# allenai/embodied-clip

Measured on AMD Instinct MI355X. Metric: env-frames/sec (CLIP encode + policy fwd/bwd + PPO update), higher is better.
Workload: dtype bf16

## Files before the change

embodied_clip_amd/csrc/api.hip:

```cpp
#include <stdlib.h>

#include "common.h"

extern "C" int ec_version(void) { return 610; }

extern "C" const char* ec_strerror(int code) {
    switch (code) {
        case EC_OK: return "ok";
        case EC_ERR_ARG: return "invalid argument (null pointer or bad enum)";
        case EC_ERR_SHAPE: return "unsupported shape for this kernel";
        case EC_ERR_LAUNCH: return "HIP kernel launch failed";
        case EC_ERR_WORKSPACE: return "workspace too small";
        case EC_ERR_ALLOC: return "host allocation failed";
        case EC_ERR_UNSUPPORTED: return "unsupported configuration";
        default: return "unknown error";
    }
}

namespace {
int env_int(const char* name, int dflt) {
    const char* e = getenv(name);
    return e ? atoi(e) : dflt;
}
EcConfig read_config() {
    EcConfig c;
    c.conv_narrow = env_int("EC_CONV_NARROW", 3);
    c.conv_rowsn = env_int("EC_CONV_ROWSN", 1);
    c.conv_big = env_int("EC_CONV_BIG", 1);
    c.conv8_min_tiles = env_int("EC_CONV8_MIN_TILES", 0);
    c.conv8_bn128 = env_int("EC_CONV8_BN128", 0);
    c.conv8_longseg = env_int("EC_CONV8_LONGSEG", 1);
    c.conv_t224 = env_int("EC_CONV_T224", 2);
    c.conv_t64 = env_int("EC_CONV_T64", 150);
    c.conv_ring = env_int("EC_CONV_RING", 1);
    c.conv_regw = env_int("EC_CONV_REGW", 1);
    c.rn50_fuse = env_int("EC_RN50_FUSE", 1);
    c.rn50_bneck = env_int("EC_RN50_BNECK", 128);
    c.rn50_bneck3 = env_int("EC_RN50_BNECK3", 1);
    c.rn50_img3 = env_int("EC_RN50_IMG3", 1);
    c.rn50_dscat = env_int("EC_RN50_DSCAT", 1);
    c.rn50_poolout = env_int("EC_RN50_POOLOUT", 1);
    c.gemm_no_x3 = env_int("EC_GEMM_NO_X3", 0);
    c.gemm_bwd3 = env_int("EC_GEMM_BWD3", 0);
    c.policy_fast = env_int("EC_POLICY_FAST", 1);
    c.act_split = env_int("EC_ACT_SPLIT", 1);
    c.tail_fused = env_int("EC_TAIL_FUSED", 1);
    c.gru_fused = env_int("EC_GRU_FUSED", 2);
    c.c1_pingpong = env_int("EC_C1_PINGPONG", 1);
    c.dw1_tr = env_int("EC_DW1_TR", 1);
    c.wih_perm = env_int("EC_WIH_PERM", 1);
    c.dw_transposed = env_int("EC_DW_TRANSPOSED", 1);
    c.vit_wide = env_int("EC_VIT_WIDE", 1);
    c.vit_bm192 = env_int("EC_VIT_BM192", 1);
    return c;
}
}

const EcConfig& ec_config() {
    static const EcConfig c = read_config();
    return c;
}

uint64_t ec_config_hash() {
    const EcConfig& c = ec_config();
    uint64_t x = 1469598103934665603ull;
    auto mix = [&](long v) {
        for (int i = 0; i < 8; ++i) { x ^= (uint64_t)((v >> (8 * i)) & 0xff); x *= 1099511628211ull; }
    };
    mix(c.conv_narrow); mix(c.conv_rowsn); mix(c.conv_big); mix(c.conv8_min_tiles); mix(c.conv8_bn128); mix(c.conv8_longseg);
    mix(c.conv_t224); mix(c.conv_t64); mix(c.conv_ring); mix(c.conv_regw); mix(c.rn50_fuse); mix(c.rn50_bneck); mix(c.rn50_bneck3);
    mix(c.rn50_img3); mix(c.rn50_dscat); mix(c.rn50_poolout); mix(c.gemm_no_x3); mix(c.gemm_bwd3); mix(c.policy_fast); mix(c.act_split); mix(c.tail_fused); mix(c.gru_fused); mix(c.c1_pingpong);
    mix(c.dw1_tr); mix(c.wih_perm); mix(c.dw_transposed);
    return x;
}

namespace {
__global__ void spin_kernel(unsigned long long ticks) {
    const unsigned long long t0 = __builtin_amdgcn_s_memrealtime();
    while (__builtin_amdgcn_s_memrealtime() - t0 < ticks) __builtin_amdgcn_s_sleep(16);
}
}

extern "C" int ec_bind_streams(ec_stream_t* streams, int n, int spin_us) {
    if (!streams || n <= 0 || spin_us <= 0 || spin_us > 100000) return EC_ERR_ARG;
    if (hipDeviceSynchronize() != hipSuccess) return EC_ERR_LAUNCH;
    for (int round = 0; round < 2; ++round)
        for (int i = 0; i < n; ++i)
            hipLaunchKernelGGL(spin_kernel, dim3(1), dim3(64), 0, (hipStream_t)streams[i], (unsigned long long)spin_us * 100ull);
    EC_CHECK_LAUNCH();
    return hipDeviceSynchronize() == hipSuccess ? EC_OK : EC_ERR_LAUNCH;
}

extern "C" int ec_stream_pair_overlap(ec_stream_t a, ec_stream_t b, int spin_us, float* ratio) {
    if (!ratio || spin_us <= 0 || spin_us > 100000 || a == b) return EC_ERR_ARG;
    hipStream_t sa = (hipStream_t)a, sb = (hipStream_t)b;
    hipEvent_t e[4];
    for (auto& ev : e)
        if (hipEventCreate(&ev) != hipSuccess) return EC_ERR_LAUNCH;
    const unsigned long long ticks = (unsigned long long)spin_us * 100ull;
    float best = 1e30f;
    int rc = EC_OK;
    for (int rep = 0; rep < 3 && rc == EC_OK; ++rep) {
        float alone = 0.f, both = 0.f;
        if (hipDeviceSynchronize() != hipSuccess) { rc = EC_ERR_LAUNCH; break; }
        (void)hipEventRecord(e[0], sa);
        hipLaunchKernelGGL(spin_kernel, dim3(1), dim3(64), 0, sa, ticks);
        (void)hipEventRecord(e[1], sa);
        if (hipDeviceSynchronize() != hipSuccess) { rc = EC_ERR_LAUNCH; break; }
        (void)hipEventRecord(e[2], sa);
        (void)hipStreamWaitEvent(sb, e[2], 0);
        hipLaunchKernelGGL(spin_kernel, dim3(1), dim3(64), 0, sa, ticks);
        hipLaunchKernelGGL(spin_kernel, dim3(1), dim3(64), 0, sb, ticks);
        (void)hipEventRecord(e[3], sb);
        (void)hipStreamWaitEvent(sa, e[3], 0);
        (void)hipEventRecord(e[1], sa);
        if (hipDeviceSynchronize() != hipSuccess) { rc = EC_ERR_LAUNCH; break; }
        if (hipEventElapsedTime(&both, e[2], e[1]) != hipSuccess) { rc = EC_ERR_LAUNCH; break; }
        (void)hipEventRecord(e[0], sa);
        hipLaunchKernelGGL(spin_kernel, dim3(1), dim3(64), 0, sa, ticks);
        (void)hipEventRecord(e[3], sa);
        if (hipDeviceSynchronize() != hipSuccess) { rc = EC_ERR_LAUNCH; break; }
        if (hipEventElapsedTime(&alone, e[0], e[3]) != hipSuccess || alone <= 0.f) { rc = EC_ERR_LAUNCH; break; }
        best = both / alone < best ? both / alone : best;
    }
    for (auto& ev : e) (void)hipEventDestroy(ev);
    if (rc == EC_OK) *ratio = best;
    return rc;
}
```

embodied_clip_amd/csrc/conv3x3_narrow.hip:

```cpp
#include <stdlib.h>

#include <type_traits>
#include <utility>

#include "common.h"

namespace {

typedef unsigned int u32x4 __attribute__((ext_vector_type(4)));
constexpr int PX = 32;
__device__ u32x4 ec_zero_page3[4];

struct N3Args {
    const uint16_t *in, *w;
    const float* bias;
    uint16_t* out;
    int H, W, ntiles;
    unsigned in_bytes = 0;
    int dbg = 0;
};

__device__ __forceinline__ float dppq_xor1(float v) {
    return __builtin_bit_cast(float, __builtin_amdgcn_update_dpp(0, __builtin_bit_cast(int, v), 0xB1, 0xF, 0xF, true));
}
__device__ __forceinline__ float dppq_xor2(float v) {
    return __builtin_bit_cast(float, __builtin_amdgcn_update_dpp(0, __builtin_bit_cast(int, v), 0x4E, 0xF, 0xF, true));
}
__device__ __forceinline__ float relu1(float x) { return __builtin_amdgcn_fmed3f(x, 0.f, __builtin_inff()); }
__device__ __forceinline__ int wunit(int n, int hh) { return ((2 * n + hh) ^ ((n >> 3) & 1)) << 4; }

template <int CIN, int COUT, bool POOL, int NW>
__global__ __launch_bounds__(NW * 64, 1) void conv3x3_narrow_kernel(N3Args p) {
    constexpr int KSTEPS = 9 * CIN / 16;
    constexpr int CB = CIN / 16;
    constexpr int FN = COUT / 32;
    constexpr int K = 9 * CIN;
    constexpr int W_BYTES = KSTEPS * COUT * 32;
    constexpr int OP = COUT * 2 + 16;
    constexpr int STG = (POOL ? PX / 4 : PX) * OP;
    extern __shared__ __attribute__((aligned(16))) unsigned char sm[];
    float* sB = reinterpret_cast<float*>(sm + W_BYTES);
    const int tid = threadIdx.x, lane = tid & 63, wave = tid >> 6;
    unsigned char* stg = sm + W_BYTES + COUT * 4 + wave * STG;
    const int px = lane & 31, h = lane >> 5;

    ec_stage_all<COUT * (K / 8), NW * 64, u32x4>(
        tid,
        [&](int idx) { return *reinterpret_cast<const u32x4*>(p.w + (long)(idx / (K / 8)) * K + (idx % (K / 8)) * 8); },
        [&](int idx, const u32x4& v) {
            const int n = idx / (K / 8), c = idx % (K / 8);
            *reinterpret_cast<u32x4*>(sm + (c >> 1) * (COUT * 32) + wunit(n, c & 1)) = v;
        });
    for (int i = tid; i < COUT; i += NW * 64) sB[i] = p.bias[i];
    __syncthreads();

    const int GW = gridDim.x * NW;
    const unsigned char* in_b = reinterpret_cast<const unsigned char*>(p.in);
    const unsigned char* zp = reinterpret_cast<const unsigned char*>(ec_zero_page3);
    const int HW = p.H * p.W;

    const int lb = (int)ec_xcd_remap(blockIdx.x, gridDim.x);
    for (int t = lb * NW + wave; t < p.ntiles; t += GW) {
        const int m = t * PX + px;
        int y, x, pix;
        if (POOL) {
            const int q = m >> 2, s2 = m & 3;
            const int Hp = p.H >> 1, Wp = p.W >> 1;
            const int b = q / (Hp * Wp);
            const int r2 = q - b * (Hp * Wp);
            const int yp = r2 / Wp;
            y = 2 * yp + (s2 >> 1);
            x = 2 * (r2 - yp * Wp) + (s2 & 1);
            pix = (b * p.H + y) * p.W + x;
        } else {
            const int b = m / HW;
            const int r2 = m - b * HW;
            y = r2 / p.W;
            x = r2 - y * p.W;
            pix = m;
        }
        const unsigned xm = (x > 0 ? 1u : 0u) | 2u | (x < p.W - 1 ? 4u : 0u);
        const unsigned msk = (y > 0 ? xm : 0u) | (xm << 3) | (y < p.H - 1 ? (xm << 6) : 0u);
        const unsigned char* base = in_b + ((long)pix * CIN + h * 8) * 2;

        f32x16_t acc[FN];
#pragma unroll
        for (int n = 0; n < FN; ++n)
#pragma unroll
            for (int r = 0; r < 16; ++r) acc[n][r] = 0.f;
        constexpr int PH = (KSTEPS + 17) / 18, PS = KSTEPS / PH;
        static_assert(PS * PH == KSTEPS, "phase split");
        auto phase = [&](auto phc) {
            constexpr int S0 = decltype(phc)::value * PS;
            u32x4 a[PS];
            [&]<int... I>(std::integer_sequence<int, I...>) {
                ((a[I] = *reinterpret_cast<const u32x4*>(
                      ((msk >> ((S0 + I) / CB)) & 1u)
                          ? base + (((((S0 + I) / CB) / 3 - 1) * p.W + (((S0 + I) / CB) % 3 - 1)) * CIN + ((S0 + I) % CB) * 16) * 2
                          : zp + h * 16)),
                 ...);
            }(std::make_integer_sequence<int, PS>{});
            __builtin_amdgcn_sched_barrier(0);
            [&]<int... I>(std::integer_sequence<int, I...>) {
                (([&] {
                     const bf16x8_t aop = __builtin_bit_cast(bf16x8_t, a[I]);
#pragma unroll
                     for (int n = 0; n < FN; ++n) {
                         const s16x8_t wf = *reinterpret_cast<const s16x8_t*>(sm + (S0 + I) * (COUT * 32) + wunit(32 * n + px, h));
                         acc[n] = __builtin_amdgcn_mfma_f32_32x32x16_bf16(__builtin_bit_cast(bf16x8_t, wf), aop, acc[n], 0, 0, 0);
                     }
                 }()),
                 ...);
            }(std::make_integer_sequence<int, PS>{});
            __builtin_amdgcn_sched_barrier(0);
        };
        [&]<int... P>(std::integer_sequence<int, P...>) { (phase(std::integral_constant<int, P>{}), ...); }
        (std::make_integer_sequence<int, PH>{});

#pragma unroll
        for (int n = 0; n < FN; ++n)
#pragma unroll
            for (int g = 0; g < 4; ++g) {
                const int lc = 32 * n + 8 * g + 4 * h;
                const float4 bv = *reinterpret_cast<const float4*>(sB + lc);
                float v0 = fmaxf(acc[n][4 * g + 0] + bv.x, 0.f), v1 = fmaxf(acc[n][4 * g + 1] + bv.y, 0.f);
                float v2 = fmaxf(acc[n][4 * g + 2] + bv.z, 0.f), v3 = fmaxf(acc[n][4 * g + 3] + bv.w, 0.f);
                if (POOL) {
                    v0 += dppq_xor1(v0); v1 += dppq_xor1(v1); v2 += dppq_xor1(v2); v3 += dppq_xor1(v3);
                    v0 += dppq_xor2(v0); v1 += dppq_xor2(v1); v2 += dppq_xor2(v2); v3 += dppq_xor2(v3);
                    if ((lane & 3) == 0) {
                        uint2 o;
                        o.x = ec_pack2(0.25f * v0, 0.25f * v1);
                        o.y = ec_pack2(0.25f * v2, 0.25f * v3);
                        *reinterpret_cast<uint2*>(stg + (px >> 2) * OP + lc * 2) = o;
                    }
                } else {
                    uint2 o;
                    o.x = ec_pack2(v0, v1);
                    o.y = ec_pack2(v2, v3);
                    *reinterpret_cast<uint2*>(stg + px * OP + lc * 2) = o;
                }
            }
        constexpr int ORows = POOL ? PX / 4 : PX;
        constexpr int ZC = COUT / 8;
        const long orow0 = (long)t * ORows;
#pragma unroll
        for (int i = 0; i < (ORows * ZC + 63) / 64; ++i) {
            const int idx = i * 64 + lane;
            if (ORows * ZC >= 64 || idx < ORows * ZC) {
                const u32x4 v = *reinterpret_cast<const u32x4*>(stg + (idx / ZC) * OP + (idx % ZC) * 16);
                *reinterpret_cast<u32x4*>(p.out + (orow0 + idx / ZC) * COUT + (idx % ZC) * 8) = v;
            }
        }
    }
}


template <int CIN, int COUT, bool POOL, int NW>
__global__ __launch_bounds__(NW * 64, 1) void conv3x3_rows_kernel(N3Args p) {
    constexpr int KSTEPS = 9 * CIN / 16, CB = CIN / 16, FN = COUT / 32, K = 9 * CIN;
    constexpr int CPP = CIN / 8;
    constexpr int PITCH = CIN * 2 + 16;
    constexpr int RW = POOL ? 16 : 30;
    constexpr int RPB = POOL ? RW * PITCH + 128 : RW * PITCH;
    constexpr int NR = POOL ? 4 : 3;
    constexpr int REGION = NR * RPB + 4 * PITCH;
    constexpr int NCH = NR * RW * CPP;
    constexpr int IT = (NCH + 63) / 64;
    constexpr int W_BYTES = KSTEPS * COUT * 32;
    constexpr int OP = COUT * 2 + 16;
    extern __shared__ __attribute__((aligned(16))) unsigned char sm[];
    float* sB = reinterpret_cast<float*>(sm + W_BYTES);
    const int tid = threadIdx.x, lane = tid & 63, wave = tid >> 6;
    unsigned char* img = sm + W_BYTES + COUT * 4 + wave * REGION;
    const int px = lane & 31, h = lane >> 5;

    ec_stage_all<COUT * (K / 8), NW * 64, u32x4>(
        tid,
        [&](int idx) { return *reinterpret_cast<const u32x4*>(p.w + (long)(idx / (K / 8)) * K + (idx % (K / 8)) * 8); },
        [&](int idx, const u32x4& v) {
            const int n = idx / (K / 8), c = idx % (K / 8);
            *reinterpret_cast<u32x4*>(sm + (c >> 1) * (COUT * 32) + wunit(n, c & 1)) = v;
        });
    for (int i = tid; i < COUT; i += NW * 64) sB[i] = p.bias[i];
    __syncthreads();

    const int GW = gridDim.x * NW;
    const int lb = (int)ec_xcd_remap(blockIdx.x, gridDim.x);
    const int nseg = POOL ? p.W / 14 : p.W / 28;
    const int nrow = POOL ? p.H / 2 : p.H;

    int f_r[IT], f_px[IT], f_lds[IT], f_goff[IT];
#pragma unroll
    for (int i = 0; i < IT; ++i) {
        const int g = i * 64 + lane;
        const int r = g / (RW * CPP), rem = g - r * (RW * CPP);
        f_r[i] = (g < NCH) ? r : -100000;
        f_px[i] = rem / CPP;
        f_lds[i] = r * RPB + (rem / CPP) * PITCH + (rem % CPP) * 16;
        f_goff[i] = ((r * p.W + rem / CPP) * CIN + (rem % CPP) * 8) * 2;
    }
    int obase;
    if (POOL) obase = ((px >> 1) & 1) * RPB + (2 * (px >> 2) + (px & 1)) * PITCH + h * 16;
    else obase = px * PITCH + h * 16;

    f32x16_t bias_acc[FN];
#pragma unroll
    for (int n = 0; n < FN; ++n)
#pragma unroll
        for (int g = 0; g < 4; ++g) {
            const float4 bv = *reinterpret_cast<const float4*>(sB + 32 * n + 8 * g + 4 * h);
            bias_acc[n][4 * g + 0] = bv.x; bias_acc[n][4 * g + 1] = bv.y; bias_acc[n][4 * g + 2] = bv.z; bias_acc[n][4 * g + 3] = bv.w;
        }

    u32x4 nxt[IT];
    const unsigned char* in_b = reinterpret_cast<const unsigned char*>(p.in);
    const unsigned char* zp = reinterpret_cast<const unsigned char*>(ec_zero_page3);
    struct Coord { int sg, rr, b; };
    auto decode = [&](int t_) {
        const int t = __builtin_amdgcn_readfirstlane(t_);
        return Coord{t % nseg, (t / nseg) % nrow, t / (nseg * nrow)};
    };
    const Coord step = decode(GW);
    auto advance = [&](Coord c) {
        c.sg += step.sg; c.rr += step.rr; c.b += step.b;
        if (c.sg >= nseg) { c.sg -= nseg; ++c.rr; }
        if (c.rr >= nrow) { c.rr -= nrow; ++c.b; }
        return c;
    };
    auto fetch = [&](Coord c) {
        const int sgi = __builtin_amdgcn_readfirstlane(c.sg), rr = __builtin_amdgcn_readfirstlane(c.rr);
        const int b = __builtin_amdgcn_readfirstlane(c.b);
        const int y0 = POOL ? 2 * rr - 1 : rr - 1, x0 = (POOL ? 14 : 28) * sgi - 1;
        const unsigned char* base = in_b + (((long)b * p.H + y0) * p.W + x0) * (CIN * 2);
        [&]<int... I>(std::integer_sequence<int, I...>) {
            (([&] {
                 const bool ok = (unsigned)(y0 + f_r[I]) < (unsigned)p.H && (unsigned)(x0 + f_px[I]) < (unsigned)p.W;
                 nxt[I] = *reinterpret_cast<const u32x4*>(ok ? base + f_goff[I] : zp);
             }()),
             ...);
        }(std::make_integer_sequence<int, IT>{});
    };

    int t = lb * NW + wave;
    if (t >= p.ntiles) return;
    Coord cn = decode(t);
    fetch(cn);
    for (;;) {
        [&]<int... I>(std::integer_sequence<int, I...>) {
            (([&] {
                 if (I * 64 + lane < NCH) *reinterpret_cast<u32x4*>(img + f_lds[I]) = nxt[I];
             }()),
             ...);
        }(std::make_integer_sequence<int, IT>{});
        const Coord cc = cn;
        t += GW;
        const bool more = t < p.ntiles;
        if (more) { cn = advance(cn); fetch(cn); }

        f32x16_t acc[FN];
        [&]<int... S>(std::integer_sequence<int, S...>) {
            (([&] {
                 constexpr int tap = S / CB, cb = S % CB, ky = tap / 3, kx = tap % 3;
                 const s16x8_t av = *reinterpret_cast<const s16x8_t*>(img + obase + ky * RPB + kx * PITCH + cb * 32);
#pragma unroll
                 for (int n = 0; n < FN; ++n) {
                     const s16x8_t wf = *reinterpret_cast<const s16x8_t*>(sm + S * (COUT * 32) + wunit(32 * n + px, h));
                     acc[n] = __builtin_amdgcn_mfma_f32_32x32x16_bf16(__builtin_bit_cast(bf16x8_t, wf),
                                                                      __builtin_bit_cast(bf16x8_t, av),
                                                                      S == 0 ? bias_acc[n] : acc[n], 0, 0, 0);
                 }
             }()),
             ...);
        }(std::make_integer_sequence<int, KSTEPS>{});

        unsigned char* stg = img;
#pragma unroll
        for (int n = 0; n < FN; ++n)
#pragma unroll
            for (int g = 0; g < 4; ++g) {
                const int lc = 32 * n + 8 * g + 4 * h;
                float v0 = relu1(acc[n][4 * g + 0]), v1 = relu1(acc[n][4 * g + 1]);
                float v2 = relu1(acc[n][4 * g + 2]), v3 = relu1(acc[n][4 * g + 3]);
                if (POOL) {
                    v0 += dppq_xor1(v0); v1 += dppq_xor1(v1); v2 += dppq_xor1(v2); v3 += dppq_xor1(v3);
                    v0 += dppq_xor2(v0); v1 += dppq_xor2(v1); v2 += dppq_xor2(v2); v3 += dppq_xor2(v3);
                    if ((lane & 3) == 0) {
                        uint2 o;
                        o.x = ec_pack2(0.25f * v0, 0.25f * v1);
                        o.y = ec_pack2(0.25f * v2, 0.25f * v3);
                        *reinterpret_cast<uint2*>(stg + (px >> 2) * OP + lc * 2) = o;
                    }
                } else {
                    uint2 o;
                    o.x = ec_pack2(v0, v1);
                    o.y = ec_pack2(v2, v3);
                    *reinterpret_cast<uint2*>(stg + px * OP + lc * 2) = o;
                }
            }
        {
            const int sgi = __builtin_amdgcn_readfirstlane(cc.sg), rr = __builtin_amdgcn_readfirstlane(cc.rr);
            const int b = __builtin_amdgcn_readfirstlane(cc.b);
            constexpr int ORows = POOL ? 7 : 28, ZC = COUT / 8;
            const long opix = POOL ? ((long)b * (p.H / 2) + rr) * (p.W / 2) + 7 * sgi : ((long)b * p.H + rr) * p.W + 28 * sgi;
#pragma unroll
            for (int i = 0; i < (ORows * ZC + 63) / 64; ++i) {
                const int idx = i * 64 + lane;
                if (idx < ORows * ZC) {
                    const u32x4 v = *reinterpret_cast<const u32x4*>(stg + (idx / ZC) * OP + (idx % ZC) * 16);
                    *reinterpret_cast<u32x4*>(p.out + (opix + idx / ZC) * COUT + (idx % ZC) * 8) = v;
                }
            }
        }
        if (!more) break;
    }
}

template <int R>
struct FragRingN { u32x4 f[R]; };
template <int CIN, int COUT, int RT, int NW, int LEADK>
__global__ __launch_bounds__(NW * 64, 1) void conv3x3_rowsN_kernel(N3Args p) {
    constexpr int KSTEPS = 9 * CIN / 16, CB = CIN / 16, FN = COUT / 32, K = 9 * CIN;
    constexpr int CPP = CIN / 8;
    constexpr int PITCH = CIN * 2 + 16;
    constexpr int RW = 30, RPB = RW * PITCH, NR = RT + 2;
    constexpr int REGION = NR * RPB + 4 * PITCH;
    constexpr int NCH = NR * RW * CPP;
    constexpr int IT = (NCH + 63) / 64;
    constexpr int W_BYTES = KSTEPS * COUT * 32;
    constexpr int OP = COUT * 2 + 16;
    constexpr int G = RT + FN;
    constexpr int RING = (LEADK + 1) * G;
    static_assert(RT * 32 * OP <= REGION, "epilogue image fits the footprint region");
    static_assert(G * LEADK <= 15, "lgkmcnt is a 4-bit counter");
    extern __shared__ __attribute__((aligned(16))) unsigned char sm[];
    float* sB = reinterpret_cast<float*>(sm + W_BYTES);
    const int tid = threadIdx.x, lane = tid & 63, wave = tid >> 6;
    unsigned char* img = sm + W_BYTES + COUT * 4 + wave * REGION;
    const int px = lane & 31, h = lane >> 5;

    ec_stage_all<COUT * (K / 8), NW * 64, u32x4>(
        tid,
        [&](int idx) { return *reinterpret_cast<const u32x4*>(p.w + (long)(idx / (K / 8)) * K + (idx % (K / 8)) * 8); },
        [&](int idx, const u32x4& v) {
            const int n = idx / (K / 8), c = idx % (K / 8);
            *reinterpret_cast<u32x4*>(sm + (c >> 1) * (COUT * 32) + wunit(n, c & 1)) = v;
        });
    for (int i = tid; i < COUT; i += NW * 64) sB[i] = p.bias[i];
    __syncthreads();

    const int GW = gridDim.x * NW;
    const int lb = (int)ec_xcd_remap(blockIdx.x, gridDim.x);
    const int nseg = p.W / 28, nrow = p.H / RT;

    int f_lds[IT];
    unsigned f_goff[IT], f_edge[IT];
#pragma unroll
    for (int i = 0; i < IT; ++i) {
        const int g = i * 64 + lane;
        const int r = g / (RW * CPP), rem = g - r * (RW * CPP), fpx = rem / CPP;
        f_edge[i] = (g >= NCH ? 16u : 0u) | (r == 0 ? 1u : 0u) | (r == NR - 1 ? 2u : 0u) | (fpx == 0 ? 4u : 0u) | (fpx == RW - 1 ? 8u : 0u);
        f_lds[i] = r * RPB + fpx * PITCH + (rem % CPP) * 16;
        f_goff[i] = (unsigned)(((r * p.W + fpx) * CIN + (rem % CPP) * 8) * 2);
    }
#if defined(__HIP_DEVICE_COMPILE__)
    const __amdgpu_buffer_rsrc_t rs_in = __builtin_amdgcn_make_buffer_rsrc((void*)p.in, 0, p.in_bytes, 0x00020000);
#endif
    const unsigned a_lds = (unsigned)(unsigned long)(__attribute__((address_space(3))) unsigned char*)img + (unsigned)(px * PITCH + h * 16);
    const unsigned w_lds0 = (unsigned)(unsigned long)(__attribute__((address_space(3))) unsigned char*)sm + (unsigned)wunit(px, h);
    constexpr int WSEG = 32768;
    struct { unsigned v[(W_BYTES + WSEG - 1) / WSEG]; } w_lds;
#pragma unroll
    for (int q = 0; q < (W_BYTES + WSEG - 1) / WSEG; ++q) w_lds.v[q] = w_lds0 + q * WSEG;

    f32x16_t bias_acc[FN];
#pragma unroll
    for (int n = 0; n < FN; ++n)
#pragma unroll
        for (int g = 0; g < 4; ++g) {
            const float4 bv = *reinterpret_cast<const float4*>(sB + 32 * n + 8 * g + 4 * h);
            bias_acc[n][4 * g + 0] = bv.x; bias_acc[n][4 * g + 1] = bv.y; bias_acc[n][4 * g + 2] = bv.z; bias_acc[n][4 * g + 3] = bv.w;
        }

    u32x4 nxt[IT];
    struct Coord { int sg, rr, b; };
    auto decode = [&](int t_) {
        const int t = __builtin_amdgcn_readfirstlane(t_);
        return Coord{t % nseg, (t / nseg) % nrow, t / (nseg * nrow)};
    };
    const Coord step = decode(GW);
    auto advance = [&](Coord c) {
        c.sg += step.sg; c.rr += step.rr; c.b += step.b;
        if (c.sg >= nseg) { c.sg -= nseg; ++c.rr; }
        if (c.rr >= nrow) { c.rr -= nrow; ++c.b; }
        return c;
    };
    auto fetch = [&](Coord c) {
        const int sgi = __builtin_amdgcn_readfirstlane(c.sg), rr = __builtin_amdgcn_readfirstlane(c.rr);
        const int b = __builtin_amdgcn_readfirstlane(c.b);
        const int y0 = RT * rr - 1, x0 = 28 * sgi - 1;
        const unsigned base = (unsigned)((((long)b * p.H + y0) * p.W + x0) * (CIN * 2));
        const unsigned tmask = 16u | (y0 < 0 ? 1u : 0u) | (y0 + NR - 1 >= p.H ? 2u : 0u) | (x0 < 0 ? 4u : 0u) |
                               (x0 + RW - 1 >= p.W ? 8u : 0u) | ((p.dbg & 1) ? 15u : 0u);
#if defined(__HIP_DEVICE_COMPILE__)
        [&]<int... I>(std::integer_sequence<int, I...>) {
            (([&] {
                 const unsigned off = (f_edge[I] & tmask) ? 0xFFFFFFF0u : base + f_goff[I];
                 nxt[I] = __builtin_amdgcn_raw_buffer_load_b128(rs_in, (int)off, 0, 0);
             }()),
             ...);
        }(std::make_integer_sequence<int, IT>{});
#endif
    };

    int t = lb * NW + wave;
    if (t >= p.ntiles) return;
    Coord cn = decode(t);
    fetch(cn);
    for (;;) {
        [&]<int... I>(std::integer_sequence<int, I...>) {
            (([&] {
                 if (I * 64 + lane < NCH && !(p.dbg & 16)) *reinterpret_cast<u32x4*>(img + f_lds[I]) = nxt[I];
             }()),
             ...);
        }(std::make_integer_sequence<int, IT>{});
        const Coord cc = cn;
        t += GW;
        const bool more = t < p.ntiles;
        if (more) { cn = advance(cn); fetch(cn); }
        asm volatile("" ::: "memory");

        f32x16_t acc[RT][FN];
        FragRingN<RING> ring;
        auto issue = [&](auto sc, auto qc) {
            constexpr int S = decltype(sc)::value, q = decltype(qc)::value;
            constexpr int tap = S / CB, cb = S % CB, ky = tap / 3, kx = tap % 3;
            constexpr int slot = (S % (LEADK + 1)) * G + q;
            const auto& wl = w_lds;
            const unsigned al = a_lds;
            if constexpr (q < RT) {
                asm volatile("ds_read_b128 %0, %1 offset:%2" : "=v"(ring.f[slot]) : "v"(al), "n"((q + ky) * RPB + kx * PITCH + cb * 32));
            } else {
                constexpr int off = S * (COUT * 32) + (q - RT) * 1024;
                asm volatile("ds_read_b128 %0, %1 offset:%2" : "=v"(ring.f[slot]) : "v"(wl.v[off / WSEG]), "n"(off % WSEG));
            }
        };
        auto issue_step = [&](auto sc) {
            [&]<int... Q>(std::integer_sequence<int, Q...>) { (issue(sc, std::integral_constant<int, Q>{}), ...); }
            (std::make_integer_sequence<int, G>{});
        };
        if (p.dbg & 4) {
#pragma unroll
            for (int i = 0; i < RT; ++i)
#pragma unroll
                for (int n = 0; n < FN; ++n) acc[i][n] = bias_acc[n];
        } else {
        [&]<int... S>(std::integer_sequence<int, S...>) { (issue_step(std::integral_constant<int, S>{}), ...); }
        (std::make_integer_sequence<int, (LEADK < KSTEPS ? LEADK : KSTEPS)>{});
        [&]<int... S>(std::integer_sequence<int, S...>) {
            (([&] {
                 if constexpr (S + LEADK < KSTEPS) issue_step(std::integral_constant<int, S + LEADK>{});
                 constexpr int ahead = (S + LEADK < KSTEPS ? LEADK : KSTEPS - 1 - S) * G;
                 asm volatile("s_waitcnt lgkmcnt(%0)" : : "n"(ahead));
                 constexpr int base = (S % (LEADK + 1)) * G;
#pragma unroll
                 for (int q = 0; q < G; ++q) asm volatile("" : "+v"(ring.f[base + q]));
#pragma unroll
                 for (int i = 0; i < RT; ++i)
#pragma unroll
                     for (int n = 0; n < FN; ++n)
                         acc[i][n] = __builtin_amdgcn_mfma_f32_32x32x16_bf16(__builtin_bit_cast(bf16x8_t, ring.f[base + RT + n]),
                                                                            __builtin_bit_cast(bf16x8_t, ring.f[base + i]),
                                                                            S == 0 ? bias_acc[n] : acc[i][n], 0, 0, 0);
             }()),
             ...);
        }(std::make_integer_sequence<int, KSTEPS>{});
        }

        unsigned char* stg = img;
        if (!(p.dbg & 8))
#pragma unroll
        for (int i = 0; i < RT; ++i)
#pragma unroll
            for (int n = 0; n < FN; ++n)
#pragma unroll
                for (int g = 0; g < 4; ++g) {
                    const int lc = 32 * n + 8 * g + 4 * h;
                    uint2 o;
                    o.x = ec_pack2(relu1(acc[i][n][4 * g + 0]), relu1(acc[i][n][4 * g + 1]));
                    o.y = ec_pack2(relu1(acc[i][n][4 * g + 2]), relu1(acc[i][n][4 * g + 3]));
                    *reinterpret_cast<uint2*>(stg + (i * 32 + px) * OP + lc * 2) = o;
                }
        {
            const int sgi = __builtin_amdgcn_readfirstlane(cc.sg), rr = __builtin_amdgcn_readfirstlane(cc.rr);
            const int b = __builtin_amdgcn_readfirstlane(cc.b);
            constexpr int ZC = COUT / 8;
            const long opix0 = ((long)b * p.H + RT * rr) * p.W + 28 * sgi;
#pragma unroll
            for (int i = 0; i < RT; ++i) {
                const long opix = opix0 + (long)i * p.W;
#pragma unroll
                for (int j = 0; j < (28 * ZC + 63) / 64; ++j) {
                    const int idx = j * 64 + lane;
                    if (idx < 28 * ZC && !(p.dbg & 2) && !(p.dbg & 32)) {
                        const u32x4 v = *reinterpret_cast<const u32x4*>(stg + (i * 32 + idx / ZC) * OP + (idx % ZC) * 16);
                        *reinterpret_cast<u32x4*>(p.out + (opix + idx / ZC) * COUT + (idx % ZC) * 8) = v;
                    }
                }
            }
        }
        if (!more) break;
    }
}

template <int CIN, int COUT, int RT, int NW, int LEADK>
int launch_rowsN(const N3Args& p, hipStream_t s) {
    constexpr int PITCH = CIN * 2 + 16, RPB = 30 * PITCH;
    constexpr size_t lds = (size_t)(9 * CIN / 16) * COUT * 32 + COUT * 4 + (size_t)NW * ((RT + 2) * RPB + 4 * PITCH);
    static_assert(lds <= 160 * 1024, "LDS budget");
    static_assert(((RT + 2) * RPB + 4 * PITCH) % 16 == 0, "image alignment");
    auto kern = conv3x3_rowsN_kernel<CIN, COUT, RT, NW, LEADK>;
    const int dbg = 0;
    N3Args q = p;
    q.dbg = dbg;
    static std::atomic<uint64_t> attr_done{0};
    if (auto attr_g_ = ec_attr_needed(attr_done)) {
        (void)hipFuncSetAttribute(reinterpret_cast<const void*>(kern), hipFuncAttributeMaxDynamicSharedMemorySize, (int)lds);
    }
    const int wgs = (p.ntiles + NW - 1) / NW < 256 ? (p.ntiles + NW - 1) / NW : 256;
    hipLaunchKernelGGL(kern, dim3((unsigned)wgs), dim3(NW * 64), lds, s, q);
    EC_CHECK_LAUNCH();
    return EC_OK;
}

template <int CIN, int COUT, bool POOL, int NW>
int launch_rows(const N3Args& p, hipStream_t s) {
    constexpr int PITCH = CIN * 2 + 16, RW = POOL ? 16 : 30, RPB = POOL ? RW * PITCH + 128 : RW * PITCH, NR = POOL ? 4 : 3;
    constexpr size_t lds = (size_t)(9 * CIN / 16) * COUT * 32 + COUT * 4 + (size_t)NW * (NR * RPB + 4 * PITCH);
    static_assert(lds <= 160 * 1024, "LDS budget");
    static_assert((NR * RPB + 4 * PITCH) % 16 == 0, "image alignment");
    auto kern = conv3x3_rows_kernel<CIN, COUT, POOL, NW>;
    static std::atomic<uint64_t> attr_done{0};
    if (auto attr_g_ = ec_attr_needed(attr_done)) {
        (void)hipFuncSetAttribute(reinterpret_cast<const void*>(kern), hipFuncAttributeMaxDynamicSharedMemorySize, (int)lds);
    }
    const int wgs = (p.ntiles + NW - 1) / NW < 256 ? (p.ntiles + NW - 1) / NW : 256;
    hipLaunchKernelGGL(kern, dim3((unsigned)wgs), dim3(NW * 64), lds, s, p);
    EC_CHECK_LAUNCH();
    return EC_OK;
}

template <int CIN, int COUT, bool POOL, int NW = 16>
int launch_n3(const N3Args& p, hipStream_t s) {
    constexpr size_t lds = (size_t)(9 * CIN / 16) * COUT * 32 + COUT * 4 + NW * (size_t)((POOL ? PX / 4 : PX) * (COUT * 2 + 16));
    static_assert(lds <= 160 * 1024, "LDS budget");
    auto kern = conv3x3_narrow_kernel<CIN, COUT, POOL, NW>;
    static std::atomic<uint64_t> attr_done{0};
    if (auto attr_g_ = ec_attr_needed(attr_done)) {
        (void)hipFuncSetAttribute(reinterpret_cast<const void*>(kern), hipFuncAttributeMaxDynamicSharedMemorySize, (int)lds);
    }
    const int wgs = (p.ntiles + NW - 1) / NW < 256 ? (p.ntiles + NW - 1) / NW : 256;
    hipLaunchKernelGGL(kern, dim3((unsigned)wgs), dim3(NW * 64), lds, s, p);
    EC_CHECK_LAUNCH();
    return EC_OK;
}

}

int ec_conv3x3_narrow(const void* in, const void* w, const float* bias, void* out, int B, int H, int W, int Cin, int Cout,
                      int pool, hipStream_t s) {
    const int mode = ec_config().conv_narrow;
    const long M = (long)B * H * W;
    if (!mode || !bias || (pool && ((H | W) & 1))) return EC_ERR_SHAPE;
    if (mode >= 3) {
        const bool fits = pool ? (W % 14 == 0) : (W % 28 == 0);
        const long nt = pool ? (long)B * (H / 2) * (W / 14) : (long)B * H * (W / 28);
        const int rowsn = ec_config().conv_rowsn;
        if (fits && !pool && rowsn && nt <= 0x7fffffffL && M * Cin * 2 < (1L << 32) - 16) {
            if (Cin == 64 && Cout == 64 && H % 2 == 0) {
                N3Args p{(const uint16_t*)in, (const uint16_t*)w, bias, (uint16_t*)out, H, W, (int)(nt / 2)};
                p.in_bytes = (unsigned)(M * Cin * 2);
                return rowsn == 3 ? launch_rowsN<64, 64, 2, 4, 3>(p, s) : launch_rowsN<64, 64, 2, 4, 2>(p, s);
            }
            if (Cin == 32 && Cout == 32 && H % 4 == 0) {
                N3Args p{(const uint16_t*)in, (const uint16_t*)w, bias, (uint16_t*)out, H, W, (int)(nt / 4)};
                p.in_bytes = (unsigned)(M * Cin * 2);
                return rowsn == 2 ? launch_rowsN<32, 32, 4, 4, 2>(p, s) : launch_rowsN<32, 32, 4, 8, 1>(p, s);
            }
        }
        if (fits && nt <= 0x7fffffffL) {
            N3Args p{(const uint16_t*)in, (const uint16_t*)w, bias, (uint16_t*)out, H, W, (int)nt};
            if (Cin == 32 && Cout == 32 && !pool) return launch_rows<32, 32, false, 16>(p, s);
            if (Cin == 32 && Cout == 64 && pool) return launch_rows<32, 64, true, 16>(p, s);
            if (Cin == 32 && Cout == 64 && !pool) return launch_rows<32, 64, false, 16>(p, s);
            if (Cin == 64 && Cout == 64 && !pool) return launch_rows<64, 64, false, 6>(p, s);
            if (Cin == 64 && Cout == 64 && pool) return launch_rows<64, 64, true, 8>(p, s);
        }
    }
    if ((M % PX) != 0 || M / PX > 0x7fffffffL) return EC_ERR_SHAPE;
    N3Args p{(const uint16_t*)in, (const uint16_t*)w, bias, (uint16_t*)out, H, W, (int)(M / PX)};
    if (Cin == 32 && Cout == 32 && !pool) return launch_n3<32, 32, false>(p, s);
    if (Cin == 32 && Cout == 64 && pool) return launch_n3<32, 64, true>(p, s);
    if (Cin == 32 && Cout == 64 && !pool) return launch_n3<32, 64, false>(p, s);
    if (mode == 2 && Cin == 64 && Cout == 64 && !pool) return launch_n3<64, 64, false>(p, s);
    if (mode == 2 && Cin == 64 && Cout == 64 && pool) return launch_n3<64, 64, true>(p, s);
    return EC_ERR_SHAPE;
}
```

Baseline: 63630.

## Overlap conv3x3 rowsN epilogue stores with next tile's MFMA k-loop

For the 64->64 rowsN conv kernel (NW==4), the previous tile's results are packed to bf16 and held in registers. Their LDS staging writes, reads and global stores are then interleaved into the next tile's MFMA k-loop, and the lgkmcnt waits are adjusted to count the extra LDS ops. The goal is to hide epilogue latency behind compute instead of running it serially after each tile. The change also removes the rowsn==3 and rowsn==2 launch variants and disables the debug flags on the pipelined path. The cost is higher register pressure from the held results, plus a delicate hand-scheduled waitcnt accounting.

```diff
diff --git a/embodied_clip_amd/csrc/api.hip b/embodied_clip_amd/csrc/api.hip
--- a/embodied_clip_amd/csrc/api.hip
+++ b/embodied_clip_amd/csrc/api.hip
@@ -2,7 +2,7 @@
 
 #include "common.h"
 
-extern "C" int ec_version(void) { return 610; }
+extern "C" int ec_version(void) { return 620; }
 
 extern "C" const char* ec_strerror(int code) {
     switch (code) {
diff --git a/embodied_clip_amd/csrc/conv3x3_narrow.hip b/embodied_clip_amd/csrc/conv3x3_narrow.hip
--- a/embodied_clip_amd/csrc/conv3x3_narrow.hip
+++ b/embodied_clip_amd/csrc/conv3x3_narrow.hip
@@ -318,8 +318,10 @@
 
 template <int R>
 struct FragRingN { u32x4 f[R]; };
-template <int CIN, int COUT, int RT, int NW, int LEADK>
-__global__ __launch_bounds__(NW * 64, 1) void conv3x3_rowsN_kernel(N3Args p) {
+typedef unsigned int u32x2 __attribute__((ext_vector_type(2)));
+constexpr int pipe_extra(int s, int t0) { return s < t0 || s >= t0 + 16 ? 0 : (((s - t0) & 7) < 4 ? 2 : 1); }
+template <int CIN, int COUT, int RT, int NW, int LEADK, bool PIPE>
+__device__ __forceinline__ void conv3x3_rowsN_body(const N3Args& p) {
     constexpr int KSTEPS = 9 * CIN / 16, CB = CIN / 16, FN = COUT / 32, K = 9 * CIN;
     constexpr int CPP = CIN / 8;
     constexpr int PITCH = CIN * 2 + 16;
@@ -333,11 +335,16 @@
     constexpr int RING = (LEADK + 1) * G;
     static_assert(RT * 32 * OP <= REGION, "epilogue image fits the footprint region");
     static_assert(G * LEADK <= 15, "lgkmcnt is a 4-bit counter");
+    constexpr int T0 = 3 * CB - LEADK;
+    static_assert(!PIPE || (RT == 2 && FN == 2 && T0 >= 0 && T0 + 16 + 2 * LEADK < KSTEPS &&
+                            G * LEADK + 2 * (LEADK + 1) <= 15), "PIPE schedule (pipe_extra) and the 4-bit lgkmcnt");
+    static_assert(!PIPE || (28 * OP <= RPB && 4 * 128 <= 4 * PITCH), "PIPE staging: footprint row 0 + the overrun tail");
     extern __shared__ __attribute__((aligned(16))) unsigned char sm[];
     float* sB = reinterpret_cast<float*>(sm + W_BYTES);
     const int tid = threadIdx.x, lane = tid & 63, wave = tid >> 6;
     unsigned char* img = sm + W_BYTES + COUT * 4 + wave * REGION;
     const int px = lane & 31, h = lane >> 5;
+    const int dbg = PIPE ? 0 : p.dbg;
 
     ec_stage_all<COUT * (K / 8), NW * 64, u32x4>(
         tid,
@@ -401,7 +408,7 @@
         const int y0 = RT * rr - 1, x0 = 28 * sgi - 1;
         const unsigned base = (unsigned)((((long)b * p.H + y0) * p.W + x0) * (CIN * 2));
         const unsigned tmask = 16u | (y0 < 0 ? 1u : 0u) | (y0 + NR - 1 >= p.H ? 2u : 0u) | (x0 < 0 ? 4u : 0u) |
-                               (x0 + RW - 1 >= p.W ? 8u : 0u) | ((p.dbg & 1) ? 15u : 0u);
+                               (x0 + RW - 1 >= p.W ? 8u : 0u) | ((dbg & 1) ? 15u : 0u);
 #if defined(__HIP_DEVICE_COMPILE__)
         [&]<int... I>(std::integer_sequence<int, I...>) {
             (([&] {
@@ -413,14 +420,62 @@
 #endif
     };
 
+    u32x2 pk[PIPE ? RT : 1][FN][4];
+    u32x4 rb[PIPE ? RT : 1][4];
+    long p_opix0 = 0;
+    constexpr int ZC = COUT / 8;
+    const unsigned stg_lds = (unsigned)(unsigned long)(__attribute__((address_space(3))) unsigned char*)img;
+    const unsigned sw_lds = stg_lds + (unsigned)((px < 28 ? px * OP : NR * RPB + (px - 28) * 128) + h * 8);
+    const unsigned sr_lds = stg_lds + (unsigned)((lane >> 3) * OP + (lane & 7) * 16);
+    uint16_t* const out_l = p.out + (lane >> 3) * COUT + (lane & 7) * 8;
+    auto epi_write = [&](auto ic, auto kc) {
+        constexpr int i = decltype(ic)::value, n = decltype(kc)::value / 4, g = decltype(kc)::value % 4;
+        const unsigned sw = sw_lds;
+        const auto& pkr = pk;
+        asm volatile("ds_write_b64 %0, %1 offset:%2" : : "v"(sw), "v"(pkr[i][n][g]), "n"(64 * n + 16 * g));
+    };
+    auto epi_read = [&](auto ic, auto jc) {
+        constexpr int i = decltype(ic)::value, j = decltype(jc)::value;
+        const unsigned sr = sr_lds;
+        auto& rbr = rb;
+        asm volatile("ds_read_b128 %0, %1 offset:%2" : "=v"(rbr[i][j]) : "v"(sr), "n"(j * 8 * OP));
+    };
+    auto epi_store = [&](auto ic, auto jc) {
+        constexpr int i = decltype(ic)::value, j = decltype(jc)::value;
+        auto& rbr = rb;
+        asm volatile("" : "+v"(rbr[i][j]));
+        if (j < 3 || lane < 32)
+            *reinterpret_cast<u32x4*>(out_l + (p_opix0 + (long)i * p.W + j * 8) * COUT) = rbr[i][j];
+    };
+    auto epi_lds = [&](auto sc) {
+        constexpr int S = decltype(sc)::value - T0;
+        if constexpr (S >= 0 && S < 16) {
+            constexpr int r = S & 7;
+            using IC = std::integral_constant<int, S / 8>;
+            if constexpr (r < 4) {
+                epi_write(IC{}, std::integral_constant<int, 2 * r>{});
+                epi_write(IC{}, std::integral_constant<int, 2 * r + 1>{});
+            } else {
+                epi_read(IC{}, std::integral_constant<int, r - 4>{});
+            }
+        }
+    };
+    auto epi_stores = [&](auto sc) {
+        constexpr int S = decltype(sc)::value, q = S - (T0 + 4 + LEADK + 1);
+        if constexpr (q >= 0 && q < 4) { epi_store(std::integral_constant<int, 0>{}, std::integral_constant<int, q>{}); __builtin_amdgcn_sched_barrier(0); }
+        if constexpr (q >= 8 && q < 12) { epi_store(std::integral_constant<int, 1>{}, std::integral_constant<int, q - 8>{}); __builtin_amdgcn_sched_barrier(0); }
+    };
+
     int t = lb * NW + wave;
     if (t >= p.ntiles) return;
     Coord cn = decode(t);
     fetch(cn);
+    bool have = false;
     for (;;) {
+        if constexpr (PIPE) asm volatile("" ::: "memory");
         [&]<int... I>(std::integer_sequence<int, I...>) {
             (([&] {
-                 if (I * 64 + lane < NCH && !(p.dbg & 16)) *reinterpret_cast<u32x4*>(img + f_lds[I]) = nxt[I];
+                 if (I * 64 + lane < NCH && !(dbg & 16)) *reinterpret_cast<u32x4*>(img + f_lds[I]) = nxt[I];
              }()),
              ...);
         }(std::make_integer_sequence<int, IT>{});
@@ -449,36 +504,62 @@
             [&]<int... Q>(std::integer_sequence<int, Q...>) { (issue(sc, std::integral_constant<int, Q>{}), ...); }
             (std::make_integer_sequence<int, G>{});
         };
-        if (p.dbg & 4) {
+        auto kloop = [&](auto epic) {
+            constexpr bool EPI = decltype(epic)::value;
+            [&]<int... S>(std::integer_sequence<int, S...>) { (issue_step(std::integral_constant<int, S>{}), ...); }
+            (std::make_integer_sequence<int, (LEADK < KSTEPS ? LEADK : KSTEPS)>{});
+            [&]<int... S>(std::integer_sequence<int, S...>) {
+                (([&] {
+                     if constexpr (S + LEADK < KSTEPS) issue_step(std::integral_constant<int, S + LEADK>{});
+                     if constexpr (EPI) epi_lds(std::integral_constant<int, S>{});
+                     constexpr int extra = [] { int e = 0; for (int s = S - LEADK; s <= S; ++s) e += pipe_extra(s, T0); return e; }();
+                     constexpr int ahead = (S + LEADK < KSTEPS ? LEADK : KSTEPS - 1 - S) * G + (EPI ? extra : 0);
+                     static_assert(ahead <= 15, "lgkmcnt is a 4-bit counter");
+                     asm volatile("s_waitcnt lgkmcnt(%0)" : : "n"(ahead));
+                     constexpr int base = (S % (LEADK + 1)) * G;
+#pragma unroll
+                     for (int q = 0; q < G; ++q) asm volatile("" : "+v"(ring.f[base + q]));
+#pragma unroll
+                     for (int i = 0; i < RT; ++i)
+#pragma unroll
+                         for (int n = 0; n < FN; ++n)
+                             acc[i][n] = __builtin_amdgcn_mfma_f32_32x32x16_bf16(__builtin_bit_cast(bf16x8_t, ring.f[base + RT + n]),
+                                                                                __builtin_bit_cast(bf16x8_t, ring.f[base + i]),
+                                                                                S == 0 ? bias_acc[n] : acc[i][n], 0, 0, 0);
+                     if constexpr (EPI) epi_stores(std::integral_constant<int, S>{});
+                 }()),
+                 ...);
+            }(std::make_integer_sequence<int, KSTEPS>{});
+        };
+        if (dbg & 4) {
 #pragma unroll
             for (int i = 0; i < RT; ++i)
 #pragma unroll
                 for (int n = 0; n < FN; ++n) acc[i][n] = bias_acc[n];
+        } else if constexpr (PIPE) {
+            if (have) kloop(std::true_type{});
+            else kloop(std::false_type{});
         } else {
-        [&]<int... S>(std::integer_sequence<int, S...>) { (issue_step(std::integral_constant<int, S>{}), ...); }
-        (std::make_integer_sequence<int, (LEADK < KSTEPS ? LEADK : KSTEPS)>{});
-        [&]<int... S>(std::integer_sequence<int, S...>) {
-            (([&] {
-                 if constexpr (S + LEADK < KSTEPS) issue_step(std::integral_constant<int, S + LEADK>{});
-                 constexpr int ahead = (S + LEADK < KSTEPS ? LEADK : KSTEPS - 1 - S) * G;
-                 asm volatile("s_waitcnt lgkmcnt(%0)" : : "n"(ahead));
-                 constexpr int base = (S % (LEADK + 1)) * G;
-#pragma unroll
-                 for (int q = 0; q < G; ++q) asm volatile("" : "+v"(ring.f[base + q]));
-#pragma unroll
-                 for (int i = 0; i < RT; ++i)
-#pragma unroll
-                     for (int n = 0; n < FN; ++n)
-                         acc[i][n] = __builtin_amdgcn_mfma_f32_32x32x16_bf16(__builtin_bit_cast(bf16x8_t, ring.f[base + RT + n]),
-                                                                            __builtin_bit_cast(bf16x8_t, ring.f[base + i]),
-                                                                            S == 0 ? bias_acc[n] : acc[i][n], 0, 0, 0);
-             }()),
-             ...);
-        }(std::make_integer_sequence<int, KSTEPS>{});
-        }
-
+            kloop(std::false_type{});
+        }
+
+        const int sgi = __builtin_amdgcn_readfirstlane(cc.sg), rr = __builtin_amdgcn_readfirstlane(cc.rr);
+        const int b = __builtin_amdgcn_readfirstlane(cc.b);
+        if constexpr (PIPE) {
+#pragma unroll
+            for (int i = 0; i < RT; ++i)
+#pragma unroll
+                for (int n = 0; n < FN; ++n)
+#pragma unroll
+                    for (int g = 0; g < 4; ++g) {
+                        pk[i][n][g].x = ec_pack2(relu1(acc[i][n][4 * g + 0]), relu1(acc[i][n][4 * g + 1]));
+                        pk[i][n][g].y = ec_pack2(relu1(acc[i][n][4 * g + 2]), relu1(acc[i][n][4 * g + 3]));
+                    }
+            p_opix0 = ((long)b * p.H + RT * rr) * p.W + 28 * sgi;
+            have = true;
+        } else {
         unsigned char* stg = img;
-        if (!(p.dbg & 8))
+        if (!(dbg & 8))
 #pragma unroll
         for (int i = 0; i < RT; ++i)
 #pragma unroll
@@ -492,9 +573,6 @@
                     *reinterpret_cast<uint2*>(stg + (i * 32 + px) * OP + lc * 2) = o;
                 }
         {
-            const int sgi = __builtin_amdgcn_readfirstlane(cc.sg), rr = __builtin_amdgcn_readfirstlane(cc.rr);
-            const int b = __builtin_amdgcn_readfirstlane(cc.b);
-            constexpr int ZC = COUT / 8;
             const long opix0 = ((long)b * p.H + RT * rr) * p.W + 28 * sgi;
 #pragma unroll
             for (int i = 0; i < RT; ++i) {
@@ -502,15 +580,36 @@
 #pragma unroll
                 for (int j = 0; j < (28 * ZC + 63) / 64; ++j) {
                     const int idx = j * 64 + lane;
-                    if (idx < 28 * ZC && !(p.dbg & 2) && !(p.dbg & 32)) {
+                    if (idx < 28 * ZC && !(dbg & 2) && !(dbg & 32)) {
                         const u32x4 v = *reinterpret_cast<const u32x4*>(stg + (i * 32 + idx / ZC) * OP + (idx % ZC) * 16);
                         *reinterpret_cast<u32x4*>(p.out + (opix + idx / ZC) * COUT + (idx % ZC) * 8) = v;
                     }
                 }
             }
         }
+        }
         if (!more) break;
     }
+    if constexpr (PIPE) {
+        [&]<int... I>(std::integer_sequence<int, I...>) {
+            (([&] {
+                 using IC = std::integral_constant<int, I>;
+                 [&]<int... Q>(std::integer_sequence<int, Q...>) { (epi_write(IC{}, std::integral_constant<int, Q>{}), ...); }
+                 (std::make_integer_sequence<int, 8>{});
+                 [&]<int... J>(std::integer_sequence<int, J...>) { (epi_read(IC{}, std::integral_constant<int, J>{}), ...); }
+                 (std::make_integer_sequence<int, 4>{});
+                 asm volatile("s_waitcnt lgkmcnt(0)");
+                 [&]<int... J>(std::integer_sequence<int, J...>) { (epi_store(IC{}, std::integral_constant<int, J>{}), ...); }
+                 (std::make_integer_sequence<int, 4>{});
+             }()),
+             ...);
+        }(std::make_integer_sequence<int, RT>{});
+    }
+}
+
+template <int CIN, int COUT, int RT, int NW, int LEADK>
+__global__ __launch_bounds__(NW * 64, 1) void conv3x3_rowsN_kernel(N3Args p) {
+    conv3x3_rowsN_body<CIN, COUT, RT, NW, LEADK, NW == 4>(p);
 }
 
 template <int CIN, int COUT, int RT, int NW, int LEADK>
@@ -575,17 +674,16 @@
     if (mode >= 3) {
         const bool fits = pool ? (W % 14 == 0) : (W % 28 == 0);
         const long nt = pool ? (long)B * (H / 2) * (W / 14) : (long)B * H * (W / 28);
-        const int rowsn = ec_config().conv_rowsn;
-        if (fits && !pool && rowsn && nt <= 0x7fffffffL && M * Cin * 2 < (1L << 32) - 16) {
+        if (fits && !pool && ec_config().conv_rowsn && nt <= 0x7fffffffL && M * Cin * 2 < (1L << 32) - 16) {
             if (Cin == 64 && Cout == 64 && H % 2 == 0) {
                 N3Args p{(const uint16_t*)in, (const uint16_t*)w, bias, (uint16_t*)out, H, W, (int)(nt / 2)};
                 p.in_bytes = (unsigned)(M * Cin * 2);
-                return rowsn == 3 ? launch_rowsN<64, 64, 2, 4, 3>(p, s) : launch_rowsN<64, 64, 2, 4, 2>(p, s);
+                return launch_rowsN<64, 64, 2, 4, 2>(p, s);
             }
             if (Cin == 32 && Cout == 32 && H % 4 == 0) {
                 N3Args p{(const uint16_t*)in, (const uint16_t*)w, bias, (uint16_t*)out, H, W, (int)(nt / 4)};
                 p.in_bytes = (unsigned)(M * Cin * 2);
-                return rowsn == 2 ? launch_rowsN<32, 32, 4, 4, 2>(p, s) : launch_rowsN<32, 32, 4, 8, 1>(p, s);
+                return launch_rowsN<32, 32, 4, 8, 1>(p, s);
             }
         }
         if (fits && nt <= 0x7fffffffL) {
```

After: 63520. No clear change (-0.2%).
